# Buildings-Lei/kv-separate

Measured on AMD Instinct MI355X. Metric: CRC32C GiB/s device-resident, batched 1 MiB blocks, 1/2/4/8 MI355X, higher is better.
Workload: dtype u8

## Files before the change

### kv-separate_amd/csrc/crc32c_device.hip

```cpp
#include <hip/hip_runtime.h>
#include <hipcub/hipcub.hpp>

#include <cstdint>
#include <cstdio>
#include <cstdlib>
#include <cstring>
#include <memory>
#include <mutex>
#include <string>
#include <vector>

#include "../../include/kvsep_crc32c.h"
#include "gf2.h"
#include "kvsep_testing.h"
#include "kvsep_internal.h"
#include "plan_size.h"
#include "route.h"
#include "concat_run.h"
#include "pack_run.h"
#include "offsets_run.h"
#include "log_run.h"
#include "chain_run.h"
#include "logw_run.h"
#include "sst_run.h"
#include "sstw_run.h"

namespace kvsep {

#include "crc32c_fold.inc"
#include "crc32c_wide.inc"
#include "crc32c_narrow.inc"
#include "crc32c_support.inc"
#include "crc32c_verdicts.inc"
#include "crc32c_concat.inc"
#include "crc32c_pack.inc"
#include "crc32c_offsets.inc"
#include "crc32c_logwalk.inc"
#include "crc32c_logchain.inc"
#include "crc32c_logframe.inc"
#include "crc32c_sstindex.inc"
#include "crc32c_sstbuild.inc"

}

using namespace kvsep;

struct CaptureSet {
  unsigned long long id = 0;
  bool held = false;
  Scratch sc;
};
constexpr size_t kDefaultCaptureSets = 4;

struct kvsep_crc32c_ctx {
  int device = 0;
  int num_cus = 0;
  DevTables* d_tabs = nullptr;
  uint64_t piece_bytes = 128 * 1024;
  bool piece_auto = true;
  int dynamic = -1;
  int kernel = 0;
  route::Settings settings() const { return {num_cus, piece_bytes, piece_auto, dynamic, route::Kernel(kernel)}; }
  uint32_t static_contig = 1;
  Scratch sc;
  std::vector<std::unique_ptr<CaptureSet>> caps;
  uint64_t res_count = 0, res_bytes = 0;
  int host_node = -1;
  bool inject_failure = false;
  bool timing = false;
  std::vector<std::pair<hipEvent_t, hipEvent_t>> ev_pending;
  std::vector<hipEvent_t> ev_pool;
  HostStaging staging;
  std::mutex mu;
};

#include "crc32c_diag.inc"

namespace {
thread_local std::string g_last_error;

int set_err(int code, const char* what, hipError_t e = hipSuccess) {
  char buf[512];
  if (e != hipSuccess)
    snprintf(buf, sizeof buf, "%s: %s (%d)", what, hipGetErrorString(e), int(e));
  else
    snprintf(buf, sizeof buf, "%s", what);
  g_last_error = buf;
  return code;
}

#define KVSEP_HIP(call)                                              \
  do {                                                               \
    hipError_t _e = (call);                                          \
    if (_e != hipSuccess) return set_err(KVSEP_EHIP, #call, _e);     \
  } while (0)

int upload_tables(kvsep_crc32c_ctx* c) {
  DevTables h;
  gf2::byte_tables(gf2::zero_bytes_map(1024), &h.z1024[0][0]);
  gf2::byte_tables(gf2::zero_bytes_map(4), &h.z4[0][0]);
  for (int j = 0; j < 6; ++j) gf2::byte_tables(gf2::zero_bytes_map(16ull << j), &h.ztree[j][0][0]);
  for (uint32_t b = 0; b < 256; ++b) h.byte1[b] = gf2::byte_table_entry(b);
  gf2::byte_tables(gf2::zero_bytes_map(c->piece_bytes), &h.zpiece[0][0]);
  for (int k = 0; k < 3; ++k) gf2::byte_tables(gf2::zero_bytes_map(kSmallPiece << k), &h.zsmall[k][0][0]);
  gf2::byte_tables(gf2::zero_bytes_map(kNarrowRow), &h.znarrow[0][0]);
  gf2::x2n_table(h.x2n);
  gf2::xinv_table(h.xinv);
  if (!c->d_tabs) KVSEP_HIP(hipMalloc(&c->d_tabs, sizeof(DevTables)));
  KVSEP_HIP(hipMemcpy(c->d_tabs, &h, sizeof(DevTables), hipMemcpyHostToDevice));
  return KVSEP_OK;
}

int quiesce(Scratch& sc) {
  if (sc.used && sc.last_use) KVSEP_HIP(hipEventSynchronize(sc.last_use));
  return KVSEP_OK;
// ... 370 lines not shown
  }
  const int rc = launch_batch_body(c, sc, s, capturing, a, base, off, len, init, expect, out, first_bad, nbad, count,
                                   total_bytes, max_len);
  if (rc && expect && !capturing) sc.vacc_dirty = true;
  return rc;
}

int launch_batch_body(kvsep_crc32c_ctx* c, Scratch& sc, hipStream_t s, bool capturing, PiecesArgs& a,
                      const void* base, const uint64_t* off, const uint64_t* len, const uint32_t* init,
                      const uint32_t* expect, uint32_t* out, uint64_t* first_bad, uint64_t* nbad, uint64_t count,
                      uint64_t total_bytes, uint64_t max_len) {
  const route::Route route = route_of(c, count, total_bytes, max_len);
  const bool planned = route.planned;
  a.base = static_cast<const uint8_t*>(base);
  a.off = off;
  a.len = len;
  a.init = init;
  a.out = out;
  a.count = count;
  a.piece_bytes = route.piece.bytes;
  a.zpiece = !planned ? nullptr : route.piece.table < 0 ? &c->d_tabs->zpiece[0][0] : &c->d_tabs->zsmall[route.piece.table][0][0];
  a.tabs = c->d_tabs;
  if (expect) {
    if (!first_bad || !nbad) {
      first_bad = reinterpret_cast<uint64_t*>(sc.verify.p);
      nbad = reinterpret_cast<uint64_t*>(sc.verify.p + 1);
    }
    if (count == 0) {
      start_words_kernel<<<1, 64, 0, s>>>(nullptr, reinterpret_cast<unsigned long long*>(first_bad),
                                          reinterpret_cast<unsigned long long*>(nbad));
      KVSEP_HIP(hipGetLastError());
    }
  }
  a.expect = expect;
  a.first_bad = reinterpret_cast<unsigned long long*>(first_bad);
  a.nbad = reinterpret_cast<unsigned long long*>(nbad);
  if (count == 0) return KVSEP_OK;
  const bool dyn = route.dyn;
  a.static_contig = c->static_contig;
  a.guided_div = 0;
  a.guided_cap = 0;
  if (dyn) {
    int rc = ensure_counter(sc, capturing);
    if (rc) return rc;
    a.work_counter = sc.counter.p;
  }
  if (planned) {
    int rc = ensure_plan(sc, count, route.pieces_needed, capturing);
    if (rc) return rc;
    a.pstart = sc.plan_blocks.q;
    a.pblk = sc.plan_pieces.p;
    a.partial = sc.plan_pieces.q;
    a.max_pieces = sc.plan_pieces.cap;
    const unsigned nb = unsigned((count + 255) / 256);
    crc32c_plan_count_kernel<<<nb, 256, 0, s>>>(len, count, a.piece_bytes, sc.plan_blocks.p, sc.plan_blocks.q,
                                                dyn ? sc.counter.p : nullptr);
    KVSEP_HIP(hipGetLastError());
    size_t tb = sc.scan_tmp.cap;
    KVSEP_HIP(hipcub::DeviceScan::InclusiveSum(sc.scan_tmp.p, tb, sc.plan_blocks.p, sc.plan_blocks.q + 1, int(count), s));
    crc32c_plan_expand_kernel<<<nb, 256, 0, s>>>(sc.plan_blocks.q, count, sc.plan_pieces.cap, sc.plan_pieces.p);
    KVSEP_HIP(hipGetLastError());
  } else {
    a.max_pieces = count;
    if (dyn) {
      start_words_kernel<<<1, 64, 0, s>>>(sc.counter.p, nullptr, nullptr);
      KVSEP_HIP(hipGetLastError());
    }
  }
  const unsigned grid = unsigned(c->num_cus);
  hipEvent_t e0 = nullptr, e1 = nullptr;
  if (c->timing) {
    e0 = take_event(c);
    e1 = take_event(c);
    if (e0 && e1) KVSEP_HIP(hipEventRecord(e0, s));
  }
  a.hint = route.hint;
  if (route.form != route::Form::Wide) {
    KVSEP_HIP(diag_verify_words(route, s, a));
    if (!diag_launch_narrow(route, grid, s, a))
      launch_narrow(route, expect != nullptr, init != nullptr, grid, s, a);
  } else {
    launch_pieces(c, planned, dyn, expect != nullptr, grid, s, a);
  }
  KVSEP_HIP(hipGetLastError());
  if (c->inject_failure) {
    c->inject_failure = false;
    if (e0) c->ev_pool.push_back(e0);
    if (e1) c->ev_pool.push_back(e1);
    return set_err(KVSEP_EHIP, "injected failure after the CRC kernel (kvsep_crc32c_ctx_inject_failure)");
  }
  if (c->timing && e0 && e1) {
    KVSEP_HIP(hipEventRecord(e1, s));
    c->ev_pending.emplace_back(e0, e1);
  }
  const unsigned cgrid = route.combine_grid;
  if (planned) {
    a.vslot_base = grid;
    if (expect) crc32c_combine_kernel<true><<<cgrid, 256, 0, s>>>(a);
    else crc32c_combine_kernel<false><<<cgrid, 256, 0, s>>>(a);
    KVSEP_HIP(hipGetLastError());
  }
  if (expect && a.vslot) {
    verify_slots_reduce_kernel<<<1, 256, 0, s>>>(a.vslot, grid + cgrid,
                                                 reinterpret_cast<unsigned long long*>(first_bad),
                                                 reinterpret_cast<unsigned long long*>(nbad));
    KVSEP_HIP(hipGetLastError());
  }
  KVSEP_HIP(diag_verify_finish(route, s, a));
  return KVSEP_OK;
}
}

namespace kvsep {
int device_batch_locked(kvsep_crc32c_ctx* c, Scratch& sc, hipStream_t s, const void* base, const uint64_t* off,
// ... 44 lines not shown
  c->host_node = kvsep_device_numa_node(device);
  diag_env(c);
  int rc = upload_tables(c);
  if (rc) {
    delete c;
    return rc;
  }
  *out = c;
  return KVSEP_OK;
}

void kvsep_crc32c_ctx_destroy(kvsep_crc32c_ctx* c) {
  if (!c) return;
  DeviceGuard dg(c->device);
  hipDeviceSynchronize();
  free_scratch(c->sc);
  for (auto& k : c->caps) free_scratch(k->sc);
  hipFree(c->d_tabs);
  for (auto& p : c->ev_pending) { hipEventDestroy(p.first); hipEventDestroy(p.second); }
  for (auto e : c->ev_pool) hipEventDestroy(e);
  release_staging(c->staging);
  diag_forget(c);
  delete c;
}

int kvsep_crc32c_ctx_set_piece_bytes(kvsep_crc32c_ctx* c, uint64_t piece_bytes) {
  if (!c || piece_bytes < 1024 || piece_bytes % 1024) return set_err(KVSEP_EINVAL, "piece_bytes must be a multiple of 1 KiB");
  std::lock_guard<std::mutex> g(c->mu);
  for (auto& k : c->caps)
    if (k->held) return set_err(KVSEP_EINVAL, "set_piece_bytes with captured graphs held: kvsep_crc32c_release_captures first");
  DeviceGuard dg(c->device);
  KVSEP_HIP(dg.err);
  KVSEP_HIP(hipDeviceSynchronize());
  c->piece_bytes = piece_bytes;
  c->piece_auto = false;
  free_plan(c->sc);
  for (auto& sc : c->staging.scratch) free_plan(sc);
  for (auto& k : c->caps) free_plan(k->sc);
  return upload_tables(c);
}

int kvsep_crc32c_ctx_set_schedule(kvsep_crc32c_ctx* c, int dynamic) {
  if (!c) return set_err(KVSEP_EINVAL, "null ctx");
  std::lock_guard<std::mutex> g(c->mu);
  c->dynamic = dynamic < 0 ? -1 : (dynamic == 1 ? 1 : 0);
  c->static_contig = dynamic == 2 ? 0 : 1;
  return KVSEP_OK;
}

int kvsep_crc32c_ctx_set_kernel(kvsep_crc32c_ctx* c, int kernel) {
  if (!c || kernel < 0 || kernel > 8) return set_err(KVSEP_EINVAL, "kernel must be 0..8");
  std::lock_guard<std::mutex> g(c->mu);
  c->kernel = kernel;
  return KVSEP_OK;
}

int kvsep_crc32c_ctx_set_host_node(kvsep_crc32c_ctx* c, int node) {
  if (!c || node < -1) return set_err(KVSEP_EINVAL, "node must be >= -1");
  std::lock_guard<std::mutex> g(c->mu);
  c->host_node = node;
  return KVSEP_OK;
}

int kvsep_crc32c_ctx_inject_failure(kvsep_crc32c_ctx* c) {
  if (!c) return set_err(KVSEP_EINVAL, "null ctx");
  const char* on = std::getenv("KVSEP_TEST_HOOKS");
  if (!on || std::strcmp(on, "1") != 0) return set_err(KVSEP_EINVAL, "fault injection needs KVSEP_TEST_HOOKS=1");
  std::lock_guard<std::mutex> g(c->mu);
  c->inject_failure = true;
  return KVSEP_OK;
}

}

namespace {
int reserve_scratch(kvsep_crc32c_ctx* c, Scratch& sc, uint64_t count, uint64_t total_bytes) {
  int rc = ensure_counter(sc);
  if (!rc) rc = ensure_verify(sc);
  if (!rc) rc = ensure_event(sc);
  if (!rc) rc = ensure_sst(sc, count);
  if (!rc) rc = ensure_vslot(sc, vslots_needed(c));
  if (!rc) rc = ensure_list(sc, count);
  if (!rc) rc = ensure_offsets(sc, count);
  if (!rc) rc = ensure_log(sc, count);
  if (!rc) rc = ensure_chain(sc, count);
  if (!rc) rc = ensure_logw(sc, count);
  if (!rc) rc = ensure_sstidx(sc, sst::runs_for(sst::runs_reserved(count), 0));
  if (!rc) rc = ensure_sstw(sc, count);
  if (rc) return rc;
  return ensure_plan(sc, count, plan::pieces_reserved(c->piece_bytes, c->piece_auto, c->num_cus, count, total_bytes));
}

int reserve_capture_sets(kvsep_crc32c_ctx* c, size_t n) {
  while (c->caps.size() < n) c->caps.emplace_back(new CaptureSet());
  for (auto& k : c->caps) {
    if (k->held) continue;
    int rc = reserve_scratch(c, k->sc, c->res_count, c->res_bytes);
    if (rc) return rc;
  }
  return KVSEP_OK;
}
}

extern "C" {

int kvsep_crc32c_reserve(kvsep_crc32c_ctx* c, uint64_t count, uint64_t total_bytes) {
// ... 1224 lines not shown
  if (nbad) *nbad = 0;
  if (!count) return KVSEP_OK;
  const uint64_t cap = std::min(bad_cap, count);
  struct Bufs {
    void* p[5] = {nullptr, nullptr, nullptr, nullptr, nullptr};
    ~Bufs() { for (void* q : p) hipFree(q); }
  } b;
  {
    DeviceGuard dg(c->device);
    KVSEP_HIP(dg.err);
    const size_t bytes[5] = {size_t(n), size_t(count * 16), size_t(count * 4), 16, size_t(std::max<uint64_t>(cap, 1) * 8)};
    for (int i = 0; i < 5; ++i)
      if (hipMalloc(&b.p[i], bytes[i]) != hipSuccess) {
        (void)hipGetLastError();
        return set_err(KVSEP_ENOMEM, "kvsep_sst_verify_list_host: device allocation failed");
      }
    auto* d_off = static_cast<uint64_t*>(b.p[1]);
    auto* d_res = static_cast<uint64_t*>(b.p[3]);
    KVSEP_HIP(hipMemcpy(b.p[0], file, n, hipMemcpyHostToDevice));
    KVSEP_HIP(hipMemcpy(d_off, off, count * 8, hipMemcpyHostToDevice));
    KVSEP_HIP(hipMemcpy(d_off + count, len, count * 8, hipMemcpyHostToDevice));
    const int rc = kvsep_sst_verify_list_device(c, nullptr, b.p[0], d_off, d_off + count, static_cast<uint32_t*>(b.p[2]),
                                                d_res, d_res + 1, cap ? static_cast<uint64_t*>(b.p[4]) : nullptr, cap,
                                                nullptr, count, total, max_len);
    if (rc) return rc;
    uint64_t res[2];
    KVSEP_HIP(hipMemcpy(res, d_res, 16, hipMemcpyDeviceToHost));
    KVSEP_HIP(hipMemcpy(out, b.p[2], count * 4, hipMemcpyDeviceToHost));
    const uint64_t k = std::min(res[1], cap);
    if (k) KVSEP_HIP(hipMemcpy(bad_idx, b.p[4], k * 8, hipMemcpyDeviceToHost));
    if (first_bad) *first_bad = res[0];
    if (nbad) *nbad = res[1];
  }
  return KVSEP_OK;
}

const char* kvsep_crc32c_kernel_name(kvsep_crc32c_ctx* c, uint64_t count, uint64_t total_bytes, uint64_t max_len) {
  if (!c) return "";
  std::lock_guard<std::mutex> g(c->mu);
  return route::kernel_name(route_of(c, count, total_bytes, max_len).form);
}

int kvsep_crc32c_plan_query(kvsep_crc32c_ctx* c, uint64_t count, uint64_t total_bytes, uint64_t max_len,
                            uint64_t* piece_bytes, uint64_t* pieces_needed, int* guided) {
  if (!c) return set_err(KVSEP_EINVAL, "null ctx");
  std::lock_guard<std::mutex> g(c->mu);
  const route::Route r = route_of(c, count, total_bytes, max_len);
  if (piece_bytes) *piece_bytes = r.piece.bytes;
  if (pieces_needed) *pieces_needed = r.pieces_needed;
  if (guided) *guided = r.dyn ? 1 : 0;
  return KVSEP_OK;
}

int kvsep_stream_read_device(kvsep_crc32c_ctx* c, void* stream, const void* src, uint64_t nbytes, uint32_t* sink) {
  if (!c || !src || !sink) return set_err(KVSEP_EINVAL, "null argument");
  hipStream_t s = static_cast<hipStream_t>(stream);
  const uint64_t n16 = nbytes / 16;
  hipEvent_t e0 = nullptr, e1 = nullptr;
  std::lock_guard<std::mutex> g(c->mu);
  DeviceGuard dg(c->device);
  KVSEP_HIP(dg.err);
  if (c->timing) {
    e0 = take_event(c);
    e1 = take_event(c);
    if (e0 && e1) KVSEP_HIP(hipEventRecord(e0, s));
  }
  if (!diag_stream_read(c, s, reinterpret_cast<uintptr_t>(src), n16, sink))
  stream_read_kernel<<<unsigned(c->num_cus), 512, 0, s>>>(reinterpret_cast<uintptr_t>(src), n16, sink);
  KVSEP_HIP(hipGetLastError());
  if (c->timing && e0 && e1) {
    KVSEP_HIP(hipEventRecord(e1, s));
    c->ev_pending.emplace_back(e0, e1);
  }
  return KVSEP_OK;
}

const char* kvsep_last_error(void) { return g_last_error.c_str(); }

}
```

### kv-separate_amd/csrc/crc32c_fold.inc

```

constexpr uint32_t kZ4Off = 131072;
constexpr uint32_t kTreeOff = 135168;
constexpr uint32_t kByteOff = 159744;
constexpr uint32_t kLdsBytes = 160768;
constexpr uint32_t kRowBytes = 1024;

struct DevTables {
  uint32_t z1024[4][256];
  uint32_t z4[4][256];
  uint32_t ztree[6][4][256];
  uint32_t byte1[256];
  uint32_t zpiece[4][256];
  uint32_t znarrow[4][256];
  uint32_t zsmall[3][4][256];
  uint32_t x2n[64];
  uint32_t xinv[16];
};
static_assert(sizeof(DevTables) == 4096 * 13 + 1024 + 256 + 64, "table layout");

struct PiecesArgs {
  const uint8_t* base;
  const uint64_t* off;
  const uint64_t* len;
  const uint32_t* init;
  uint32_t* out;
  uint64_t count;
  const uint64_t* pstart;
  const uint32_t* pblk;
  uint32_t* partial;
  uint32_t* work_counter;
  uint64_t piece_bytes;
  const uint32_t* zpiece;
  uint64_t max_pieces;
  uint32_t static_contig;
  uint32_t guided_div;
  uint32_t guided_cap;
  uint64_t hint;
  const uint32_t* expect;
  unsigned long long* first_bad;
  unsigned long long* nbad;
  const DevTables* tabs;
  unsigned long long* vacc;
  unsigned long long* vslot;
  uint32_t vslot_base;
};

template <typename T>
__device__ __forceinline__ T ldc(const T* p, uint64_t i) {
  return reinterpret_cast<const __attribute__((address_space(4))) T*>(reinterpret_cast<uintptr_t>(p))[i];
}

__device__ __forceinline__ uint32_t lds_u32(const uint8_t* lds, uint32_t byte_off) {
  return *reinterpret_cast<const uint32_t*>(lds + byte_off);
}

__device__ __forceinline__ uint32_t xor3(uint32_t a, uint32_t b, uint32_t c) {
  return __builtin_amdgcn_bitop3_b32(a, b, c, 0x96);
}

__device__ __forceinline__ uint32_t zmap(const uint8_t* lds, uint32_t t, uint32_t w) {
  return lds_u32(lds, t + ((w << 2) & 0x3fcu)) ^ lds_u32(lds, t + 1024u + ((w >> 6) & 0x3fcu)) ^
         lds_u32(lds, t + 2048u + ((w >> 14) & 0x3fcu)) ^ lds_u32(lds, t + 3072u + ((w >> 22) & 0x3fcu));
}

__device__ __forceinline__ uint32_t zmap_x(const uint8_t* lds, uint32_t t, uint32_t w, uint32_t x) {
  return xor3(xor3(lds_u32(lds, t + ((w << 2) & 0x3fcu)), lds_u32(lds, t + 1024u + ((w >> 6) & 0x3fcu)), x),
              lds_u32(lds, t + 2048u + ((w >> 14) & 0x3fcu)), lds_u32(lds, t + 3072u + ((w >> 22) & 0x3fcu)));
}

__device__ __forceinline__ uint32_t fold1024(const uint8_t* lds, uint32_t c, uint32_t lc0, uint32_t lc1) {
  const uint32_t a0 = __builtin_amdgcn_perm(c, lc0, 0x0C020400u);
  const uint32_t a1 = __builtin_amdgcn_perm(c, lc0, 0x0C020500u);
  const uint32_t a2 = __builtin_amdgcn_perm(c, lc1, 0x0C020600u);
  const uint32_t a3 = __builtin_amdgcn_perm(c, lc1, 0x0C020700u);
  return lds_u32(lds, a0) ^ lds_u32(lds, a1 + 128u) ^ lds_u32(lds, a2) ^ lds_u32(lds, a3 + 128u);
}

__device__ __forceinline__ uint32_t fold_step(const uint8_t* lds, uint32_t c, uint32_t w, uint32_t lc0, uint32_t lc1) {
  const uint32_t a0 = __builtin_amdgcn_perm(c, lc0, 0x0C020400u);
  const uint32_t a1 = __builtin_amdgcn_perm(c, lc0, 0x0C020500u);
  const uint32_t a2 = __builtin_amdgcn_perm(c, lc1, 0x0C020600u);
  const uint32_t a3 = __builtin_amdgcn_perm(c, lc1, 0x0C020700u);
  return xor3(xor3(lds_u32(lds, a0), lds_u32(lds, a1 + 128u), w), lds_u32(lds, a2), lds_u32(lds, a3 + 128u));
}

template <int N>
__device__ __forceinline__ uint32_t row_shr(uint32_t v) {
  return uint32_t(__builtin_amdgcn_update_dpp(0, int(v), 0x110 + N, 0xF, 0xF, false));
}

__device__ __forceinline__ uint4 uniform4(uint4 v) {
  return make_uint4(uint32_t(__builtin_amdgcn_readfirstlane(int(v.x))), uint32_t(__builtin_amdgcn_readfirstlane(int(v.y))),
                    uint32_t(__builtin_amdgcn_readfirstlane(int(v.z))), uint32_t(__builtin_amdgcn_readfirstlane(int(v.w))));
}

__device__ __forceinline__ uint32_t serial16(const uint8_t* lds, uint32_t reg, uint4 ch, int q0, int q1,
                                             uint32_t z4 = kZ4Off, uint32_t byte = kByteOff) {
  const uint32_t w[4] = {ch.x, ch.y, ch.z, ch.w};
// ... 501 lines not shown
```

### kv-separate_amd/csrc/crc32c_support.inc

```

template <bool kVerify = false>
__global__ void __launch_bounds__(256) crc32c_combine_kernel(PiecesArgs a) {
  __shared__ uint32_t zp[1024];
  for (uint32_t i = threadIdx.x; i < 1024; i += 256) zp[i] = a.zpiece[i];
  __syncthreads();
#ifdef KVSEP_DIAG
  {
    const uintptr_t p[6] = {uintptr_t(a.pstart), uintptr_t(a.partial), uintptr_t(a.out), uintptr_t(a.expect),
                            uintptr_t(a.vslot), uintptr_t(a.vslot_base)};
    for (int i = 0; i < 6; ++i)
      if (i == 5 ? a.vslot_base > 4096u : (p[i] >> 47) != 0) {
        if (threadIdx.x == 0)
          printf("KVSEP combine: wg %u arg %d = %p (pstart %p partial %p out %p expect %p vslot %p count %llu max %llu)\n",
                 blockIdx.x, i, (void*)p[i], (void*)p[0], (void*)p[1], (void*)p[2], (void*)p[3], (void*)p[4],
                 (unsigned long long)a.count, (unsigned long long)a.max_pieces);
        return;
      }
  }
#endif
  const bool fallback = a.pstart[a.count] > a.max_pieces;
  VAcc vacc;
  for (uint64_t b0 = uint64_t(blockIdx.x) * 256; b0 < a.count; b0 += uint64_t(gridDim.x) * 256) {
    const uint64_t b = b0 + threadIdx.x;
    const uint64_t bb = b < a.count ? b : a.count - 1;
    uint64_t s = a.pstart[bb], e = a.pstart[bb + 1];
#ifdef KVSEP_DIAG
    if (b < a.count && !fallback && (e < s || e > a.max_pieces)) {
      printf("KVSEP combine: wg %u block %llu of %llu: pieces [%llu, %llu) of %llu (pstart %p: %llx %llx .. %llx)\n",
             blockIdx.x, (unsigned long long)b, (unsigned long long)a.count, (unsigned long long)s,
             (unsigned long long)e, (unsigned long long)a.max_pieces, (void*)a.pstart,
             (unsigned long long)a.pstart[0], (unsigned long long)a.pstart[1], (unsigned long long)a.pstart[a.count]);
      s = e = 0;
    }
#endif
    const bool mine = b < a.count && e - s > 1 && !fallback;
    uint32_t crc = 0;
    if (mine) {
      uint32_t acc = a.partial[s];
      for (uint64_t g = s + 1; g < e; ++g) {
        acc = zp[acc & 255u] ^ zp[256 + ((acc >> 8) & 255u)] ^ zp[512 + ((acc >> 16) & 255u)] ^ zp[768 + (acc >> 24)];
        acc ^= a.partial[g];
      }
      crc = ~acc;
      emit_block(a, b, crc);
    }
    if (kVerify) verify_wave(vacc, mine, b0, threadIdx.x, crc, ld32(a.expect + bb));
  }
  if (kVerify) verify_publish<4, kVaccShards>(a, threadIdx.x >> 6, vacc);
}

__global__ void start_words_kernel(uint32_t* w32, unsigned long long* first_bad, unsigned long long* nbad) {
  if (threadIdx.x == 0) {
    if (w32) *w32 = 0;
    if (first_bad) *first_bad = ~0ull;
    if (nbad) *nbad = 0;
  }
}

__global__ void __launch_bounds__(256) verify_slots_reduce_kernel(const unsigned long long* vslot, uint32_t n,
                                                                  unsigned long long* first_bad,
                                                                  unsigned long long* nbad) {
  __shared__ unsigned long long sb[256], sn[256];
  unsigned long long b = ~0ull, c = 0;
#ifdef KVSEP_DIAG
  if ((uintptr_t(vslot) >> 47) || (uintptr_t(first_bad) >> 47) || (uintptr_t(nbad) >> 47) || n > 4096u) {
    if (threadIdx.x == 0) printf("KVSEP reduce: vslot %p n %u first_bad %p nbad %p\n", vslot, n, first_bad, nbad);
    return;
  }
#endif
  for (uint32_t i = threadIdx.x; i < n; i += 256) {
    const unsigned long long x = vslot[2ull * i];
    b = x < b ? x : b;
    c += vslot[2ull * i + 1];
  }
  sb[threadIdx.x] = b;
  sn[threadIdx.x] = c;
  __syncthreads();
  for (uint32_t h = 128; h; h >>= 1) {
// ... 115 lines not shown
```

### kv-separate_amd/csrc/crc32c_wide.inc

```

template <bool kPlanned, bool kDynamic, int kG, bool kNT, bool kAhead, int kThreads = kWgThreads, bool kAlign = true,
          bool kVerify = false, typename Ext = Exact>
__global__ void __launch_bounds__(kThreads) crc32c_pieces_kernel(PiecesArgs a) {
  constexpr uint32_t kWavesPerWg = kThreads / 64;
  constexpr bool kPad = Ext::kPad;
  __shared__ __attribute__((aligned(16))) uint8_t lds[kLdsBytes];
  const uint32_t tid = threadIdx.x;
  KVSEP_WSTAMP_ENTRY();
  const uint32_t lane = tid & 63u;
  uint32_t vz;
  asm volatile("v_mov_b32 %0, 0" : "=v"(vz));
  const uint32_t lc0 = (lane & 31u) << 2;
  const uint32_t lc1 = lc0 | 0x10000u;
  const uint32_t wave = __builtin_amdgcn_readfirstlane(tid >> 6);
  const uint64_t nwaves = uint64_t(gridDim.x) * kWavesPerWg;

  uint64_t total = a.count;
  bool planned = kPlanned;
  if (kPlanned) {
    total = ldc(a.pstart, a.count);
    if (total > a.max_pieces) {
      planned = false;
      total = a.count;
    }
  }

  uint64_t lo = ~uint64_t(0), hi = 0;
  uint64_t seen = 0;
  uint64_t gdiv = a.guided_div;
  if (!gdiv) {
    gdiv = total / (64 * nwaves);
    gdiv = gdiv < 4 ? 4 : gdiv > 32 ? 32 : gdiv;
  }
  auto grab = [&]() -> bool {
    if (kDynamic) {
      const uint64_t rem = total > seen ? total - seen : 0;
      uint64_t c = rem / (gdiv * nwaves);
      if (a.guided_cap && c > a.guided_cap) c = a.guided_cap;
      if (c < 1) c = 1;
      if (c > 0xffffffffull) c = 0xffffffffull;
      uint32_t t = 0;
      if (lane == 0) t = atomicAdd(a.work_counter, uint32_t(c));
      lo = uint32_t(__builtin_amdgcn_readfirstlane(t));
      hi = lo + c < total ? lo + c : total;
      seen = lo + c;
    } else if (a.static_contig) {
      if (lo != ~uint64_t(0)) return false;
      const uint64_t per = (total + nwaves - 1) / nwaves;
      lo = (uint64_t(wave) * gridDim.x + blockIdx.x) * per;
      hi = lo + per < total ? lo + per : total;
    } else {
      lo = (lo == ~uint64_t(0)) ? uint64_t(wave) * gridDim.x + blockIdx.x : lo + nwaves;
      hi = lo + 1;
    }
    return lo < total;
  };

  uint64_t w0 = 0, wn = 0;
  uintptr_t w_ps = 0, w_pe = 0;
  uint32_t w_b = 0, w_reg0 = 0, w_only = 0, w_exp = 0;
  auto fill_set = [&](uint64_t start, uint64_t n, uintptr_t& w_ps, uintptr_t& w_pe, uint32_t& w_b, uint32_t& w_reg0,
                      uint32_t& w_only, uint32_t& w_exp) {
    const uint64_t g = start + lane;
    w_ps = w_pe = 0;
    w_b = w_reg0 = w_only = w_exp = 0;
    if (g < start + n) {
      uint64_t b, rs, re;
      bool first, only;
      if (planned) {
        b = a.pblk[g];
        const uint64_t s0 = a.pstart[b], k = a.pstart[b + 1] - s0, j = g - s0;
        const uint64_t n = a.len[b];
        re = n - (k - 1 - j) * a.piece_bytes;
        rs = j ? n - (k - j) * a.piece_bytes : 0;
        first = (j == 0);
        only = (k == 1);
      } else {
        b = g;
        rs = 0;
        re = a.len[b];
        first = true;
        only = true;
      }
      const uintptr_t blk = reinterpret_cast<uintptr_t>(a.base) + a.off[b];
      w_ps = blk + rs;
      w_pe = blk + re;
      w_b = uint32_t(b);
      w_reg0 = first ? ~(a.init ? a.init[b] : 0u) : 0u;
      if (kPad && w_ps < w_pe && (w_ps & 15u) && w_reg0)
        w_reg0 = gf2_mulmod(a.tabs->xinv[w_ps & 15u], w_reg0);
      w_only = only ? 1u : 0u;
      if (kVerify) w_exp = only ? a.expect[b] : 0u;
    }
  };
  auto fill = [&](uint64_t start, uint64_t stop) {
    w0 = start;
    const uint64_t left = stop - start;
    wn = left < 64 ? left : 64;
    fill_set(w0, wn, w_ps, w_pe, w_b, w_reg0, w_only, w_exp);
  };
  struct Item {
    uint64_t g, b;
    uint32_t reg0, exp;
    bool only;
  };
  auto take = [&](uint64_t g, Item& it, Staged<kG>& st) {
    const uint32_t i = uint32_t(g - w0);
    auto rl = [i](uint32_t v) -> uint32_t { return uint32_t(__builtin_amdgcn_readlane(int(v), int(i))); };
    it.g = g;
    it.b = rl(w_b);
    it.reg0 = rl(w_reg0);
    it.only = rl(w_only) != 0;
    it.exp = kVerify ? rl(w_exp) : 0u;
    const uintptr_t ps = (uintptr_t(rl(uint32_t(w_ps >> 32))) << 32) | uintptr_t(rl(uint32_t(w_ps)));
    const uintptr_t pe = (uintptr_t(rl(uint32_t(w_pe >> 32))) << 32) | uintptr_t(rl(uint32_t(w_pe)));
    stage<kG, kNT, kAlign, kPad>(st, ps, pe, lane, reinterpret_cast<uintptr_t>(a.tabs), vz);
  };
  VAcc vacc;
  auto emit = [&](const Item& it, uint32_t reg) {
    if (lane == 0) {
      if (it.only) emit_block(a, it.b, ~reg);
      else a.partial[it.g] = reg;
    }
    if (kVerify && it.only) verify_uniform(vacc, it.b, ~uint32_t(__builtin_amdgcn_readlane(int(reg), 0)), it.exp);
  };

  auto step = [&](uint64_t g, uint64_t end, Item& ia, Staged<kG>& A, Item& ib, Staged<kG>& B) {
    const bool hn = g + 1 < end;
    KVSEP_WSTAMP_ITEM_BEGIN();
// ... 29 lines not shown
```

### kv-separate_amd/csrc/kvsep_testing.h

```cpp
#pragma once

#include "../../include/kvsep_crc32c.h"

#ifdef __cplusplus
extern "C" {
#endif

int kvsep_crc32c_ctx_inject_failure(kvsep_crc32c_ctx* ctx);

int kvsep_crc32c_plan_query(kvsep_crc32c_ctx* ctx, uint64_t count, uint64_t total_bytes, uint64_t max_len,
                            uint64_t* piece_bytes, uint64_t* pieces_needed, int* guided);

#ifdef __cplusplus
}
#endif
```

### kv-separate_amd/csrc/route.h

```cpp
#pragma once
#include <algorithm>
#include <cstdint>

#include "plan_size.h"

namespace kvsep {

constexpr int kWgThreads = 512;
static_assert(kWgThreads / 64 == kPlanWavesPerWg, "plan_size.h sizes plans for the default CRC workgroup");

constexpr uint64_t kNarrowMax = 32 * 1024;
constexpr uint64_t kCoopMaxLen = 4096;

constexpr uint32_t kCombineMaxGrid = 2048;

constexpr uint32_t kClaimLean = 3;

namespace route {

enum class Kernel : int {
  Auto = 0,
  Wide = 1,
  Narrow = 2,
  Narrow16 = 3,
  Narrow8 = 4,
  Sorted = 5,
  Claim = 6,
  Claim16 = 7,
  Coop = 8,
};

struct Settings {
  int num_cus;
  uint64_t piece_bytes;
  bool piece_auto;
  int dynamic;
  Kernel kernel;
};

enum class Form : int {
  Wide = 0,
  Narrow16 = 6,
  Narrow8 = 9,
  Claim = 10,
  Claim16 = 11,
  Coop = 12,
  Sorted = 20,
};

inline const char* kernel_name(Form f) {
  switch (f) {
    case Form::Wide: return "crc32c_pieces_kernel";
    case Form::Sorted: return "crc32c_narrow_sorted_kernel";
    case Form::Claim:
    case Form::Claim16: return "crc32c_narrow_claim_kernel";
    case Form::Coop: return "crc32c_narrow_coop_kernel";
    default: return "crc32c_narrow_kernel";
  }
}

constexpr int kDiagNone = 1;

struct Route {
  bool planned;
  plan::Piece piece;
  bool dyn;
  Form form;
  uint64_t hint;
  unsigned threads;
  unsigned combine_grid;
  uint64_t pieces_needed;
  int variant;
};

inline Route decide(const Settings& s, uint64_t count, uint64_t total_bytes, uint64_t max_len, int diag = kDiagNone) {
  Route r;
  r.planned = !(max_len != 0 && max_len <= s.piece_bytes);
  r.piece = r.planned ? plan::piece_for(s.piece_bytes, s.piece_auto, s.num_cus, total_bytes)
                      : plan::Piece{s.piece_bytes, -1};
  r.pieces_needed = r.planned ? plan::pieces_needed(r.piece.bytes, count, total_bytes) : 0;
  r.combine_grid = r.planned ? unsigned(std::min<uint64_t>((count + 255) / 256, kCombineMaxGrid)) : 0u;
  const uint64_t est_items = r.planned ? count + total_bytes / r.piece.bytes : count;
  const uint64_t nwaves_est = uint64_t(s.num_cus) * (kWgThreads / 64);
  r.dyn = s.dynamic < 0 ? (r.planned && est_items >= 8 * nwaves_est) : s.dynamic == 1;
  r.form = Form::Wide;
  r.hint = 0;
  r.threads = kWgThreads;
  r.variant = kDiagNone;

  const bool ragged = count != 0 && total_bytes != 0 && 4 * max_len > 5 * (total_bytes / count);

  const uint64_t bytes = total_bytes ? total_bytes : count * max_len;
  const bool claim16 = max_len >= 8 * 1024 && max_len <= 12 * 1024 && count >= 4096 && bytes <= (512ull << 20);

  if (r.planned || max_len > 2 * kNarrowMax || s.kernel == Kernel::Wide) return r;
  if (s.kernel == Kernel::Auto) {
    const uint64_t cus = uint64_t(s.num_cus);
    const bool enough = (claim16 && !ragged) || (max_len <= 8 * 1024 && count >= 32 * cus) ||
                        (max_len <= 16 * 1024 && count >= 64 * cus) || (max_len <= kNarrowMax && count >= 128 * cus);
    if (diag == 0 || (diag < 2 && !enough)) return r;
  }

  switch (s.kernel) {
    case Kernel::Narrow16: r.form = Form::Narrow16; break;
    case Kernel::Narrow8: r.form = Form::Narrow8; break;
    case Kernel::Sorted: r.form = Form::Sorted; break;
    case Kernel::Claim: r.form = Form::Claim; break;
    case Kernel::Claim16: r.form = Form::Claim16; break;
    case Kernel::Coop: r.form = Form::Coop; break;
    default:
      if (ragged) r.form = Form::Sorted;
      else if (claim16) r.form = Form::Claim16;
      else if (max_len <= 8 * 1024 && count >= (1u << 15) && count <= (max_len <= 4 * 1024 ? 3u << 17 : 1u << 16))
        r.form = Form::Claim;
      else if (max_len <= 8 * 1024 ? count >= (1u << 17) : count >= (1u << 15)) r.form = Form::Narrow8;
      else r.form = Form::Narrow16;
      if (diag != kDiagNone && diag != 7) {
        const bool shipped = diag == 6 || diag == 9 || diag == 10 || diag == 11 || diag == 20;
        r.form = shipped ? Form(diag) : Form::Narrow16;
        if (!shipped) r.variant = diag;
      }
  }
  r.hint = max_len;
  if (r.form == Form::Coop) r.hint = std::min(r.hint, kCoopMaxLen);
  if (r.form == Form::Narrow16 || r.form == Form::Sorted) r.threads = 1024;
  return r;
}

}
}
```

### kv-separate_amd/kvsep/__init__.py

```python
from __future__ import annotations

import ctypes
import os
import re
import sys

try:
    import torch
except Exception:
    torch = None

import numpy as np

_HERE = os.path.dirname(os.path.abspath(__file__))
LIB_PATH = os.path.join(_HERE, "libkvsep_crc32c.so")
HEADER_PATH = os.path.join(_HERE, "..", "..", "include", "kvsep_crc32c.h")

KVSEP_OK = 0
MASK_DELTA = 0xA282EAD8
OFFSET_SKIP = 2**64 - 1

_lib = None


class KvsepError(RuntimeError):
    pass


def _u32p():
    return ctypes.POINTER(ctypes.c_uint32)


def _u64p():
    return ctypes.POINTER(ctypes.c_uint64)


_SIGS = {
    "kvsep_crc32c_extend": (ctypes.c_uint32, [ctypes.c_uint32, ctypes.c_void_p, ctypes.c_size_t]),
    "kvsep_crc32c_value": (ctypes.c_uint32, [ctypes.c_void_p, ctypes.c_size_t]),
    "kvsep_crc32c_mask": (ctypes.c_uint32, [ctypes.c_uint32]),
    "kvsep_crc32c_unmask": (ctypes.c_uint32, [ctypes.c_uint32]),
    "kvsep_accelerated_crc32c": (ctypes.c_uint32, [ctypes.c_uint32, ctypes.c_void_p, ctypes.c_size_t]),
    "kvsep_set_offload_threshold": (None, [ctypes.c_uint64]),
    "kvsep_set_offload_wait": (None, [ctypes.c_int]),
    "kvsep_offload_stats": (None, [ctypes.c_void_p, ctypes.c_void_p, ctypes.c_void_p]),
    "kvsep_crc32c_kernel_name": (ctypes.c_char_p, [ctypes.c_void_p, ctypes.c_uint64, ctypes.c_uint64, ctypes.c_uint64]),
    "kvsep_crc32c_extend_host": (ctypes.c_uint32, [ctypes.c_uint32, ctypes.c_void_p, ctypes.c_size_t]),
    "kvsep_crc32c_host_path": (ctypes.c_char_p, []),
    "kvsep_crc32c_ctx_set_host_node": (ctypes.c_int, [ctypes.c_void_p, ctypes.c_int]),
    "kvsep_crc32c_ctx_host_placement": (ctypes.c_int, [ctypes.c_void_p, ctypes.c_void_p, ctypes.c_void_p,
                                                       ctypes.c_void_p, ctypes.c_int]),
    "kvsep_crc32c_ctx_inject_failure": (ctypes.c_int, [ctypes.c_void_p]),
    "kvsep_crc32c_plan_query": (ctypes.c_int, [ctypes.c_void_p, ctypes.c_uint64, ctypes.c_uint64, ctypes.c_uint64,
                                               ctypes.POINTER(ctypes.c_uint64), ctypes.POINTER(ctypes.c_uint64),
                                               ctypes.POINTER(ctypes.c_int)]),
    "kvsep_device_pci_bus_id": (ctypes.c_int, [ctypes.c_int, ctypes.c_char_p, ctypes.c_int]),
    "kvsep_pci_numa_node": (ctypes.c_int, [ctypes.c_char_p]),
    "kvsep_device_numa_node": (ctypes.c_int, [ctypes.c_int]),
    "kvsep_numa_node_cpus": (ctypes.c_int, [ctypes.c_int, ctypes.c_void_p, ctypes.c_int]),
    "kvsep_bind_process_numa": (ctypes.c_int, [ctypes.c_int]),
    "kvsep_host_page_node": (ctypes.c_int, [ctypes.c_void_p]),
    "kvsep_crc32c_ctx_create": (ctypes.c_int, [ctypes.c_int, ctypes.POINTER(ctypes.c_void_p)]),
    "kvsep_crc32c_ctx_destroy": (None, [ctypes.c_void_p]),
    "kvsep_crc32c_ctx_set_piece_bytes": (ctypes.c_int, [ctypes.c_void_p, ctypes.c_uint64]),
    "kvsep_crc32c_ctx_set_schedule": (ctypes.c_int, [ctypes.c_void_p, ctypes.c_int]),
    "kvsep_crc32c_ctx_set_kernel": (ctypes.c_int, [ctypes.c_void_p, ctypes.c_int]),
    "kvsep_crc32c_reserve": (ctypes.c_int, [ctypes.c_void_p, ctypes.c_uint64, ctypes.c_uint64]),
    "kvsep_crc32c_reserve_captures": (ctypes.c_int, [ctypes.c_void_p, ctypes.c_int]),
    "kvsep_crc32c_release_captures": (ctypes.c_int, [ctypes.c_void_p]),
    "kvsep_crc32c_capture_sets": (ctypes.c_int, [ctypes.c_void_p, ctypes.POINTER(ctypes.c_int)]),
    "kvsep_crc32c_ctx_set_timing": (ctypes.c_int, [ctypes.c_void_p, ctypes.c_int]),
    "kvsep_crc32c_ctx_get_timing": (ctypes.c_int, [ctypes.c_void_p, ctypes.POINTER(ctypes.c_double),
                                                   ctypes.POINTER(ctypes.c_uint64)]),
    "kvsep_crc32c_batch_device": (ctypes.c_int, [ctypes.c_void_p, ctypes.c_void_p, ctypes.c_void_p, ctypes.c_void_p,
                                                 ctypes.c_void_p, ctypes.c_void_p, ctypes.c_void_p, ctypes.c_uint64,
                                                 ctypes.c_uint64, ctypes.c_uint64]),
    "kvsep_crc32c_verify_device": (ctypes.c_int, [ctypes.c_void_p, ctypes.c_void_p, ctypes.c_void_p, ctypes.c_void_p,
                                                  ctypes.c_void_p, ctypes.c_void_p, ctypes.c_void_p, ctypes.c_void_p,
                                                  ctypes.c_void_p, ctypes.c_void_p, ctypes.c_uint64, ctypes.c_uint64,
                                                  ctypes.c_uint64]),
    "kvsep_crc32c_verify_list_device": (ctypes.c_int, [ctypes.c_void_p] * 11 + [ctypes.c_uint64, ctypes.c_void_p,
                                                       ctypes.c_uint64, ctypes.c_uint64, ctypes.c_uint64]),
    "kvsep_sst_verify_list_device": (ctypes.c_int, [ctypes.c_void_p] * 9 + [ctypes.c_uint64, ctypes.c_void_p,
                                                    ctypes.c_uint64, ctypes.c_uint64, ctypes.c_uint64]),
    "kvsep_sst_verify_list_host": (ctypes.c_int, [ctypes.c_void_p, ctypes.c_void_p, ctypes.c_uint64] +
                                   [ctypes.c_void_p] * 6 + [ctypes.c_uint64, ctypes.c_uint64]),
    "kvsep_log_verify_device": (ctypes.c_int, [ctypes.c_void_p] * 7 + [ctypes.c_uint64, ctypes.c_uint64,
                                               ctypes.c_uint64]),
    "kvsep_crc32c_group_verify_list_device": (ctypes.c_int, [ctypes.c_void_p] * 14 + [ctypes.c_uint64]),
    "kvsep_crc32c_combine": (ctypes.c_uint32, [ctypes.c_uint32, ctypes.c_uint32, ctypes.c_uint64]),
    "kvsep_crc32c_concat_device": (ctypes.c_int, [ctypes.c_void_p] * 7 + [ctypes.c_uint64, ctypes.c_uint64]),
    "kvsep_crc32c_gather_device": (ctypes.c_int, [ctypes.c_void_p] * 9 + [ctypes.c_uint64] * 4),
    "kvsep_crc32c_gather_host": (ctypes.c_int, [ctypes.c_void_p] * 6 + [ctypes.c_uint64, ctypes.c_uint64]),
    "kvsep_crc32c_pack_device": (ctypes.c_int, [ctypes.c_void_p] * 7 + [ctypes.c_uint64, ctypes.c_void_p,
                                                ctypes.c_uint64, ctypes.c_uint64]),
    "kvsep_vlog_frame_offsets": (ctypes.c_int, [ctypes.c_void_p, ctypes.c_uint64, ctypes.c_uint64, ctypes.c_void_p,
                                                ctypes.c_void_p]),
    "kvsep_vlog_frame_device": (ctypes.c_int, [ctypes.c_void_p] * 9 + [ctypes.c_uint64, ctypes.c_void_p] +
                                [ctypes.c_uint64] * 4),
    "kvsep_sst_frame_device": (ctypes.c_int, [ctypes.c_void_p] * 8 + [ctypes.c_uint64, ctypes.c_void_p] +
                               [ctypes.c_uint64] * 3),
    "kvsep_crc32c_offsets_device": (ctypes.c_int, [ctypes.c_void_p] * 6 + [ctypes.c_uint64] * 3 +
                                    [ctypes.c_void_p] * 3 + [ctypes.c_uint64] * 2),
    "kvsep_crc32c_salvage_device": (ctypes.c_int, [ctypes.c_void_p] * 8 + [ctypes.c_uint64] + [ctypes.c_void_p] * 3 +
                                    [ctypes.c_uint64]),
    "kvsep_sst_salvage_device": (ctypes.c_int, [ctypes.c_void_p] * 10 + [ctypes.c_uint64] + [ctypes.c_void_p] * 3 +
                                 [ctypes.c_uint64] * 3),
    "kvsep_vlog_frame_auto_device": (ctypes.c_int, [ctypes.c_void_p] * 9 + [ctypes.c_uint64] * 2 +
# ... 218 lines not shown
            pass

    def set_piece_bytes(self, n: int):
        _check(lib().kvsep_crc32c_ctx_set_piece_bytes(self._h, n), "set_piece_bytes")

    def set_schedule(self, dynamic):
        v = -1 if dynamic is None else 2 if dynamic == "rr" else (1 if dynamic else 0)
        _check(lib().kvsep_crc32c_ctx_set_schedule(self._h, v), "set_schedule")

    KERNELS = {"auto": 0, "wide": 1, "narrow": 2, "narrow16": 3, "narrow8": 4, "sorted": 5, "claim": 6, "claim16": 7,
               "coop": 8}

    def set_kernel(self, kernel: str):
        _check(lib().kvsep_crc32c_ctx_set_kernel(self._h, self.KERNELS[kernel]), "set_kernel")

    def set_host_node(self, node: int):
        _check(lib().kvsep_crc32c_ctx_set_host_node(self._h, node), "set_host_node")

    def host_placement(self):
        dn, sn = ctypes.c_int(), ctypes.c_int()
        cpus = (ctypes.c_int * 4096)()
        n = lib().kvsep_crc32c_ctx_host_placement(self._h, ctypes.byref(dn), ctypes.byref(sn), cpus, 4096)
        if n < 0:
            _check(n, "host_placement")
        return {"device_node": dn.value, "staging_node": sn.value, "copier_cpus": list(cpus[:min(n, 4096)])}

    def inject_failure(self):
        _check(lib().kvsep_crc32c_ctx_inject_failure(self._h), "inject_failure")

    def reserve(self, count: int, total_bytes: int):
        _check(lib().kvsep_crc32c_reserve(self._h, count, total_bytes), "reserve")

    def reserve_captures(self, nsets: int):
        _check(lib().kvsep_crc32c_reserve_captures(self._h, nsets), "reserve_captures")

    def release_captures(self):
        _check(lib().kvsep_crc32c_release_captures(self._h), "release_captures")

    def capture_sets(self):
        held = ctypes.c_int(0)
        n = lib().kvsep_crc32c_capture_sets(self._h, ctypes.byref(held))
        _check(n if n < 0 else 0, "capture_sets")
        return n, held.value

    def kernel_name(self, count: int, max_len: int, total_bytes: int = 0) -> str:
        return lib().kvsep_crc32c_kernel_name(self._h, count, total_bytes, max_len).decode()

    def plan_query(self, count: int, max_len: int, total_bytes: int = 0):
        pb, pn, gd = ctypes.c_uint64(), ctypes.c_uint64(), ctypes.c_int()
        _check(lib().kvsep_crc32c_plan_query(self._h, count, total_bytes, max_len, ctypes.byref(pb), ctypes.byref(pn),
                                             ctypes.byref(gd)), "plan_query")
        return pb.value, pn.value, bool(gd.value)

    def set_timing(self, on: bool):
        _check(lib().kvsep_crc32c_ctx_set_timing(self._h, 1 if on else 0), "set_timing")

    def get_timing(self):
        ms = ctypes.c_double()
        n = ctypes.c_uint64()
        _check(lib().kvsep_crc32c_ctx_get_timing(self._h, ctypes.byref(ms), ctypes.byref(n)), "get_timing")
        return ms.value, n.value

    def batch_device(self, base, off, length, out, init=None, count=None, total_bytes=None, max_len=0, stream=None):
        count = int(off.numel()) if count is None else count
        if total_bytes is None:
            total_bytes = int(length.sum().item()) if count else 0
        _check(lib().kvsep_crc32c_batch_device(self._h, _stream_handle(stream), _dptr(base), _dptr(off),
                                               _dptr(length), _dptr(init), _dptr(out), count, total_bytes,
                                               max_len), "kvsep_crc32c_batch_device")
        return out

    def verify_device(self, base, off, length, expected_masked, out, first_bad, nbad, init=None, count=None,
                      total_bytes=None, max_len=0, stream=None):
        count = int(off.numel()) if count is None else count
        if total_bytes is None:
            total_bytes = int(length.sum().item()) if count else 0
        _check(lib().kvsep_crc32c_verify_device(self._h, _stream_handle(stream), _dptr(base), _dptr(off),
                                                _dptr(length), _dptr(init), _dptr(expected_masked), _dptr(out),
                                                _dptr(first_bad), _dptr(nbad), count, total_bytes, max_len),
               "kvsep_crc32c_verify_device")
        return out

    def verify_list_device(self, base, off, length, expected_masked, out, first_bad, nbad, bad_idx=None, bad_cap=None,
                           ok=None, init=None, count=None, total_bytes=None, max_len=0, stream=None):
        count = int(off.numel()) if count is None else count
        if total_bytes is None:
            total_bytes = int(length.sum().item()) if count else 0
        if bad_cap is None:
            bad_cap = 0 if bad_idx is None else int(bad_idx.numel())
        _check(lib().kvsep_crc32c_verify_list_device(self._h, _stream_handle(stream), _dptr(base), _dptr(off),
                                                     _dptr(length), _dptr(init), _dptr(expected_masked), _dptr(out),
                                                     _dptr(first_bad), _dptr(nbad), _dptr(bad_idx), bad_cap, _dptr(ok),
                                                     count, total_bytes, max_len),
               "kvsep_crc32c_verify_list_device")
        return out

    def log_verify_device(self, base, off, length, stored, ok, count=None, total_bytes=None, max_len=0, stream=None):
        count = int(off.numel()) if count is None else count
        if total_bytes is None:
            total_bytes = int(length.sum().item()) if count else 0
        _check(lib().kvsep_log_verify_device(self._h, _stream_handle(stream), _dptr(base), _dptr(off), _dptr(length),
                                             _dptr(stored), _dptr(ok), count, total_bytes, max_len),
               "kvsep_log_verify_device")
        return ok

    def log_walk_device(self, base, n, nrec, off=None, length=None, stored=None, type=None, cap=None, stream=None):
# ... 759 lines not shown
```

Measured before the change: 6494.

## Replace explicit piece plan with implicit fixed-slot mapping for uniform batches

Adds an implicit plan mode where each block gets a fixed number of piece slots (max_len / piece_bytes). Piece index to block and offset then come from a division instead of a count kernel, a hipcub scan and an expand kernel. This removes three launches and the plan-table loads per call when the total is under 8 GiB and the piece size is a power of two. The cost is launching empty slots for blocks shorter than max_len and a per-piece integer divide.

```diff
diff --git a/kv-separate_amd/csrc/crc32c_device.hip b/kv-separate_amd/csrc/crc32c_device.hip
--- a/kv-separate_amd/csrc/crc32c_device.hip
+++ b/kv-separate_amd/csrc/crc32c_device.hip
@@ -60,7 +60,10 @@
   bool piece_auto = true;
   int dynamic = -1;
   int kernel = 0;
-  route::Settings settings() const { return {num_cus, piece_bytes, piece_auto, dynamic, route::Kernel(kernel)}; }
+  int plan_mode = 0;
+  route::Settings settings() const {
+    return {num_cus, piece_bytes, piece_auto, dynamic, route::Kernel(kernel), route::PlanMode(plan_mode)};
+  }
   uint32_t static_contig = 1;
   Scratch sc;
   std::vector<std::unique_ptr<CaptureSet>> caps;
@@ -537,14 +540,22 @@
     a.pblk = sc.plan_pieces.p;
     a.partial = sc.plan_pieces.q;
     a.max_pieces = sc.plan_pieces.cap;
-    const unsigned nb = unsigned((count + 255) / 256);
-    crc32c_plan_count_kernel<<<nb, 256, 0, s>>>(len, count, a.piece_bytes, sc.plan_blocks.p, sc.plan_blocks.q,
-                                                dyn ? sc.counter.p : nullptr);
-    KVSEP_HIP(hipGetLastError());
-    size_t tb = sc.scan_tmp.cap;
-    KVSEP_HIP(hipcub::DeviceScan::InclusiveSum(sc.scan_tmp.p, tb, sc.plan_blocks.p, sc.plan_blocks.q + 1, int(count), s));
-    crc32c_plan_expand_kernel<<<nb, 256, 0, s>>>(sc.plan_blocks.q, count, sc.plan_pieces.cap, sc.plan_pieces.p);
-    KVSEP_HIP(hipGetLastError());
+    a.slots = route.slots;
+    if (route.slots) {
+      if (dyn) {
+        start_words_kernel<<<1, 64, 0, s>>>(sc.counter.p, nullptr, nullptr);
+        KVSEP_HIP(hipGetLastError());
+      }
+    } else {
+      const unsigned nb = unsigned((count + 255) / 256);
+      crc32c_plan_count_kernel<<<nb, 256, 0, s>>>(len, count, a.piece_bytes, sc.plan_blocks.p, sc.plan_blocks.q,
+                                                  dyn ? sc.counter.p : nullptr);
+      KVSEP_HIP(hipGetLastError());
+      size_t tb = sc.scan_tmp.cap;
+      KVSEP_HIP(hipcub::DeviceScan::InclusiveSum(sc.scan_tmp.p, tb, sc.plan_blocks.p, sc.plan_blocks.q + 1, int(count), s));
+      crc32c_plan_expand_kernel<<<nb, 256, 0, s>>>(sc.plan_blocks.q, count, sc.plan_pieces.cap, sc.plan_pieces.p);
+      KVSEP_HIP(hipGetLastError());
+    }
   } else {
     a.max_pieces = count;
     if (dyn) {
@@ -695,6 +706,13 @@
   if (!c || kernel < 0 || kernel > 8) return set_err(KVSEP_EINVAL, "kernel must be 0..8");
   std::lock_guard<std::mutex> g(c->mu);
   c->kernel = kernel;
+  return KVSEP_OK;
+}
+
+int kvsep_crc32c_ctx_set_plan_mode(kvsep_crc32c_ctx* c, int mode) {
+  if (!c || mode < 0 || mode > 2) return set_err(KVSEP_EINVAL, "plan mode must be 0..2");
+  std::lock_guard<std::mutex> g(c->mu);
+  c->plan_mode = mode;
   return KVSEP_OK;
 }
 
@@ -2025,6 +2043,15 @@
   return KVSEP_OK;
 }
 
+int kvsep_crc32c_plan_slots_query(kvsep_crc32c_ctx* c, uint64_t count, uint64_t total_bytes, uint64_t max_len,
+                                  uint32_t* slots, int* mode) {
+  if (!c) return set_err(KVSEP_EINVAL, "null ctx");
+  std::lock_guard<std::mutex> g(c->mu);
+  if (slots) *slots = route_of(c, count, total_bytes, max_len).slots;
+  if (mode) *mode = c->plan_mode;
+  return KVSEP_OK;
+}
+
 int kvsep_stream_read_device(kvsep_crc32c_ctx* c, void* stream, const void* src, uint64_t nbytes, uint32_t* sink) {
   if (!c || !src || !sink) return set_err(KVSEP_EINVAL, "null argument");
   hipStream_t s = static_cast<hipStream_t>(stream);
diff --git a/kv-separate_amd/csrc/crc32c_fold.inc b/kv-separate_amd/csrc/crc32c_fold.inc
--- a/kv-separate_amd/csrc/crc32c_fold.inc
+++ b/kv-separate_amd/csrc/crc32c_fold.inc
@@ -43,7 +43,14 @@
   unsigned long long* vacc;
   unsigned long long* vslot;
   uint32_t vslot_base;
-};
+  uint32_t slots;
+};
+static_assert(sizeof(PiecesArgs) == 184, "slots fills the padding after vslot_base: no field moved");
+
+__device__ __forceinline__ uint64_t implicit_pieces(uint64_t n, uint64_t piece_bytes, uint32_t slots) {
+  const uint64_t k = n < 2 * piece_bytes ? 1u : n >> __builtin_ctzll(piece_bytes);
+  return k < slots ? k : slots;
+}
 
 template <typename T>
 __device__ __forceinline__ T ldc(const T* p, uint64_t i) {
diff --git a/kv-separate_amd/csrc/crc32c_support.inc b/kv-separate_amd/csrc/crc32c_support.inc
--- a/kv-separate_amd/csrc/crc32c_support.inc
+++ b/kv-separate_amd/csrc/crc32c_support.inc
@@ -18,12 +18,20 @@
       }
   }
 #endif
-  const bool fallback = a.pstart[a.count] > a.max_pieces;
+  const uint64_t slots = a.slots;
+  const bool fallback = (slots ? a.count * slots : a.pstart[a.count]) > a.max_pieces;
   VAcc vacc;
   for (uint64_t b0 = uint64_t(blockIdx.x) * 256; b0 < a.count; b0 += uint64_t(gridDim.x) * 256) {
     const uint64_t b = b0 + threadIdx.x;
     const uint64_t bb = b < a.count ? b : a.count - 1;
-    uint64_t s = a.pstart[bb], e = a.pstart[bb + 1];
+    uint64_t s, e;
+    if (slots) {
+      s = bb * slots;
+      e = s + implicit_pieces(a.len[bb], a.piece_bytes, a.slots);
+    } else {
+      s = a.pstart[bb];
+      e = a.pstart[bb + 1];
+    }
 #ifdef KVSEP_DIAG
     if (b < a.count && !fallback && (e < s || e > a.max_pieces)) {
       printf("KVSEP combine: wg %u block %llu of %llu: pieces [%llu, %llu) of %llu (pstart %p: %llx %llx .. %llx)\n",
diff --git a/kv-separate_amd/csrc/crc32c_wide.inc b/kv-separate_amd/csrc/crc32c_wide.inc
--- a/kv-separate_amd/csrc/crc32c_wide.inc
+++ b/kv-separate_amd/csrc/crc32c_wide.inc
@@ -18,7 +18,7 @@
   uint64_t total = a.count;
   bool planned = kPlanned;
   if (kPlanned) {
-    total = ldc(a.pstart, a.count);
+    total = a.slots ? a.count * a.slots : ldc(a.pstart, a.count);
     if (total > a.max_pieces) {
       planned = false;
       total = a.count;
@@ -68,13 +68,29 @@
       uint64_t b, rs, re;
       bool first, only;
       if (planned) {
-        b = a.pblk[g];
-        const uint64_t s0 = a.pstart[b], k = a.pstart[b + 1] - s0, j = g - s0;
+        uint32_t slots = a.slots;
+        asm volatile("" : "+s"(slots));
+        uint64_t k, j;
+        if (slots) {
+          const uint32_t q = uint32_t(g) / slots;
+          b = q;
+          j = uint32_t(g) - q * slots;
+        } else {
+          b = a.pblk[g];
+        }
         const uint64_t n = a.len[b];
-        re = n - (k - 1 - j) * a.piece_bytes;
-        rs = j ? n - (k - j) * a.piece_bytes : 0;
+        if (slots) {
+          k = implicit_pieces(n, a.piece_bytes, slots);
+        } else {
+          const uint64_t s0 = a.pstart[b];
+          k = a.pstart[b + 1] - s0;
+          j = g - s0;
+        }
+        const bool empty = j >= k;
+        re = empty ? 0 : n - (k - 1 - j) * a.piece_bytes;
+        rs = j && !empty ? n - (k - j) * a.piece_bytes : 0;
         first = (j == 0);
-        only = (k == 1);
+        only = (k == 1) && !empty;
       } else {
         b = g;
         rs = 0;
diff --git a/kv-separate_amd/csrc/kvsep_testing.h b/kv-separate_amd/csrc/kvsep_testing.h
--- a/kv-separate_amd/csrc/kvsep_testing.h
+++ b/kv-separate_amd/csrc/kvsep_testing.h
@@ -11,6 +11,11 @@
 int kvsep_crc32c_plan_query(kvsep_crc32c_ctx* ctx, uint64_t count, uint64_t total_bytes, uint64_t max_len,
                             uint64_t* piece_bytes, uint64_t* pieces_needed, int* guided);
 
+int kvsep_crc32c_ctx_set_plan_mode(kvsep_crc32c_ctx* ctx, int mode);
+
+int kvsep_crc32c_plan_slots_query(kvsep_crc32c_ctx* ctx, uint64_t count, uint64_t total_bytes, uint64_t max_len,
+                                  uint32_t* slots, int* mode);
+
 #ifdef __cplusplus
 }
 #endif
diff --git a/kv-separate_amd/csrc/route.h b/kv-separate_amd/csrc/route.h
--- a/kv-separate_amd/csrc/route.h
+++ b/kv-separate_amd/csrc/route.h
@@ -30,12 +30,19 @@
   Coop = 8,
 };
 
+enum class PlanMode : int {
+  Auto = 0,
+  Explicit = 1,
+  Implicit = 2,
+};
+
 struct Settings {
   int num_cus;
   uint64_t piece_bytes;
   bool piece_auto;
   int dynamic;
   Kernel kernel;
+  PlanMode plan_mode = PlanMode::Auto;
 };
 
 enum class Form : int {
@@ -70,6 +77,7 @@
   unsigned threads;
   unsigned combine_grid;
   uint64_t pieces_needed;
+  uint32_t slots;
   int variant;
 };
 
@@ -87,6 +95,14 @@
   r.hint = 0;
   r.threads = kWgThreads;
   r.variant = kDiagNone;
+
+  r.slots = 0;
+  const bool pow2 = (r.piece.bytes & (r.piece.bytes - 1)) == 0;
+  const bool wanted = s.plan_mode == PlanMode::Implicit || (s.plan_mode == PlanMode::Auto && total_bytes < (8ull << 30));
+  if (r.planned && pow2 && wanted && max_len != 0 && count != 0) {
+    const uint64_t k = std::max<uint64_t>(1, max_len / r.piece.bytes);
+    if (k >= 2 && k <= 0xffffffffull && k <= (count + total_bytes / r.piece.bytes) / count) r.slots = uint32_t(k);
+  }
 
   const bool ragged = count != 0 && total_bytes != 0 && 4 * max_len > 5 * (total_bytes / count);
 
diff --git a/kv-separate_amd/kvsep/__init__.py b/kv-separate_amd/kvsep/__init__.py
--- a/kv-separate_amd/kvsep/__init__.py
+++ b/kv-separate_amd/kvsep/__init__.py
@@ -54,6 +54,9 @@
     "kvsep_crc32c_plan_query": (ctypes.c_int, [ctypes.c_void_p, ctypes.c_uint64, ctypes.c_uint64, ctypes.c_uint64,
                                                ctypes.POINTER(ctypes.c_uint64), ctypes.POINTER(ctypes.c_uint64),
                                                ctypes.POINTER(ctypes.c_int)]),
+    "kvsep_crc32c_ctx_set_plan_mode": (ctypes.c_int, [ctypes.c_void_p, ctypes.c_int]),
+    "kvsep_crc32c_plan_slots_query": (ctypes.c_int, [ctypes.c_void_p, ctypes.c_uint64, ctypes.c_uint64, ctypes.c_uint64,
+                                                     ctypes.POINTER(ctypes.c_uint32), ctypes.POINTER(ctypes.c_int)]),
     "kvsep_device_pci_bus_id": (ctypes.c_int, [ctypes.c_int, ctypes.c_char_p, ctypes.c_int]),
     "kvsep_pci_numa_node": (ctypes.c_int, [ctypes.c_char_p]),
     "kvsep_device_numa_node": (ctypes.c_int, [ctypes.c_int]),
@@ -378,6 +381,17 @@
                                              ctypes.byref(gd)), "plan_query")
         return pb.value, pn.value, bool(gd.value)
 
+    PLAN_MODES = {"auto": 0, "explicit": 1, "implicit": 2}
+
+    def set_plan_mode(self, mode: str):
+        _check(lib().kvsep_crc32c_ctx_set_plan_mode(self._h, self.PLAN_MODES[mode]), "set_plan_mode")
+
+    def plan_slots(self, count: int, max_len: int, total_bytes: int = 0):
+        sl, md = ctypes.c_uint32(), ctypes.c_int()
+        _check(lib().kvsep_crc32c_plan_slots_query(self._h, count, total_bytes, max_len, ctypes.byref(sl),
+                                                   ctypes.byref(md)), "plan_slots")
+        return sl.value, {v: k for k, v in self.PLAN_MODES.items()}[md.value]
+
     def set_timing(self, on: bool):
         _check(lib().kvsep_crc32c_ctx_set_timing(self._h, 1 if on else 0), "set_timing")
 
```

Result: no change. 6523, median of 2 (+0.4%).
